# SqueezeAILab/SqueezeLLM

Measured on AMD Instinct MI355X. Metric: LLaMA-7B-shaped quantised-linear decode throughput (batch 1, all QuantLinearLUT matvecs of the model per token), higher is better.
Workload: dtype f32; 1 GPU; llama-7b w4 s0 (dense-only), batch=1 decode, 32 layers x 7 linears, op vecquant4matmul_nuq_perchannel; config_name=7b-w4-s0, launch=graph, linears sharing an input (q/k/v, gate/up) fused into one launch each, parallelism=single GPU, world_size=1, rccl_ranks=0

## Files before the change

### squeezellm_amd/csrc/sqllm_capi.hip

```cpp
#include <hip/hip_runtime.h>
#include <stdint.h>
#include <string.h>

#include <atomic>

#include "sqllm_hip.h"
#include "sqllm_host.h"
#include "sqllm_kernels.h"

namespace sqllm {
hipError_t (*g_launch_linear_gated)(int bits, const LaunchArgs& a, void* pair, hipStream_t stream) = nullptr;
hipError_t (*g_launch_linear_ep)(int bits, const LaunchArgs& a, const void* residual, int act, hipStream_t stream) = nullptr;
}

namespace sqllm_host {

ExperimentalHooks g_experimental;
static Knobs g_knobs[kMaxDevices];

int device_slot() {
  int dev = 0;
  if (hipGetDevice(&dev) != hipSuccess) {
    (void)hipGetLastError();
    dev = 0;
// ... 160 lines not shown
  const int resident = table > 3 ? table : 3;
  if (batch > 5 || total <= resident * cu_count() || (gm[0].sparse_last & 1)) return false;
  int sparse = 0;
  for (int i = 0; i < n; ++i) sparse += gm[i].csr_blocks + gm[i].topx_blocks;
  if (4 * sparse < 5 * cu_count()) return false;
  for (int i = 0; i < n; ++i)
    if (gm[i].csr_blocks > 0) {
      gm[i].csr_wide = 1;
      gm[i].csr_blocks = (gm[i].nnz + 2 * sqllm::kCsrChunk - 1) / (2 * sqllm::kCsrChunk);
      place_dense(&gm[i]);
    }
  return true;
}

void fill_segment(const sqllm_op* op, sqllm::Segment* sg) {
  sg->q = reinterpret_cast<const uint32_t*>(op->qweight);
  sg->y = op->mul;
  sg->lut = op->lookup_table;
  sg->rows = op->rows;
  sg->cols = op->cols;
  sg->vals = op->vals;
  sg->full_rows = op->topX > 0 ? op->full_rows : nullptr;
  sg->full_idx = op->topX > 0 ? op->full_row_indices : nullptr;
  sg->bias = nullptr;
  sg->out16 = nullptr;
}

static void cut_ranges(sqllm::KernelGeom* gm, int bits, int ops_in_launch, int step, int target, int grid_y) {
  const long long total_units = (long long)gm->col_tiles * gm->units_total;
  long long upw = (long long)opt(&Knobs::groups_per_wave) * step;
  bool aligned = false;
  if (upw <= 0) {
    if (opt(&Knobs::target_wgs) > 0) target = opt(&Knobs::target_wgs);
    target = (target + ops_in_launch - 1) / ops_in_launch;
    long long ranges = (target + grid_y - 1) / grid_y;
    if (ranges < 1) ranges = 1;
    upw = (total_units + ranges - 1) / ranges;
    const long long upws = (upw + step - 1) / step * step;
    const long long need = (gm->units_total + upws - 1) / upws;
    for (long long per_tile = need; per_tile >= 1 && per_tile >= need - 1 && !aligned; --per_tile) {
      long long even = (gm->units_total + per_tile - 1) / per_tile;
      even = (even + step - 1) / step * step;
      const long long n_even = (long long)gm->col_tiles * ((gm->units_total + even - 1) / even);
      if (n_even <= ranges && 10 * n_even >= 9 * ranges) { upw = even; aligned = true; }
    }
    if (aligned && ops_in_launch >= 3 && bits == 4 && gm->nnz > 0 && (gm->units_total + upw - 1) / upw == 3 &&
        gm->units_total % upw != 0 && gm->units_total % (2 * sqllm::kWaves) == 0)
      upw = gm->units_total / 2;
  }
  upw = (upw + step - 1) / step * step;
  if (upw > 0x3fffffff) upw = 0x3fffffff / step * step;
  gm->units_per_wg = (int)upw;
  gm->k_slices = (int)((gm->units_total + upw - 1) / upw);
  gm->dense_blocks = aligned ? gm->col_tiles * gm->k_slices : (int)((total_units + upw - 1) / upw);
  gm->sparse_last = 0;
  place_dense(gm);
}

void make_plan_mfma(const sqllm_op* op, sqllm::KernelGeom* gm, int ops_in_launch = 1, int row_blocks = 0, int wgs_per_cu = 0, int reserve = 0) {
  make_plan(op, gm, 1);
  const int mb = row_blocks > 0 ? row_blocks : sqllm::mfma_row_blocks(gm->batch);
  int target = (wgs_per_cu > 0 ? wgs_per_cu : mb == 4 ? 1 : 2) * cu_count();
  if (reserve > 0 && target - reserve >= target / 2) target -= reserve;
  cut_ranges(gm, op->bits, ops_in_launch, sqllm::kWaves * 4, target, (gm->batch + 16 * mb - 1) / (16 * mb));
}

constexpr int kWideTiles = 8;
int make_plan_wide(const sqllm_op* op, sqllm::KernelGeom* gm) {
  make_plan(op, gm, 1);
  const int row_blocks = (gm->batch + 63) / 64;
  const int col_groups = (gm->col_tiles + kWideTiles - 1) / kWideTiles;
  const long long units = (long long)col_groups * row_blocks;
  const int cus = cu_count();
  const long long full = units / cus * cus;
  const long long rem = units - full;
  int max_s = gm->units_total / (op->bits == 4 ? 32 : 8);
  if (max_s > sqllm::kMaxSlices) max_s = sqllm::kMaxSlices;
  if (max_s < 1) max_s = 1;
  int s = rem > 0 ? (int)(cus / rem) : 1;
  if (s > max_s) s = max_s;
  if (s < 1) s = 1;
  const int want = opt(&Knobs::groups_per_wave) * 4;
  int upw = want > 0 ? want : ((gm->units_total + s - 1) / s + 3) / 4 * 4;
  if (upw > gm->units_total) upw = (gm->units_total + 3) / 4 * 4;
  gm->units_per_wg = upw;
  gm->k_slices = (gm->units_total + upw - 1) / upw;
  const long long blocks = full + rem * gm->k_slices;
  gm->dense_blocks = blocks > 0x7fffffff ? 0x7fffffff : (int)blocks;
  gm->sparse_last = 0;
  place_dense(gm);
  return (int)full;
}

bool takes_wide_path(const sqllm_op* op, bool with_scratch, bool capturing) {
  if (!opt(&Knobs::mfma_split)) return false;
  const int from = opt(&Knobs::mfma_wide_min_batch);
  if (from > 0) return op->batch >= from;
  if (op->batch < 64) return false;
  if (with_scratch) {
    const double work = (double)op->batch * op->K * op->N;
    return work >= (op->bits == 4 ? 5.7e9 : 4e9) * (capturing ? 3.0 : 1.0);
  }
  const long long col_groups = ((op->N + sqllm::kTileN - 1) / sqllm::kTileN + kWideTiles - 1) / kWideTiles;
  const long long units = col_groups * ((op->batch + 63) / 64);
  return 5 * units >= 4 * (long long)cu_count();
}

void fold_csr_into_dense(sqllm::KernelGeom* gm) {
  gm->fold_csr = gm->nnz > 0 ? 1 : 0;
  gm->csr_blocks = 0;
  place_dense(gm);
}

int small_topx_blocks(const sqllm_op* op, bool with_xT, int ops_in_launch) {
  if (!(op->full_rows && op->topX > 0)) return 0;
  const int slabs = (op->K + sqllm::kTopxRows - 1) / sqllm::kTopxRows;
  if (!with_xT || op->topX > 16) return slabs;
  const int want = ops_in_launch == 1 ? (slabs <= 24 ? 24 : 16) : slabs <= 40 ? 8 : 16;
  return slabs < want ? slabs : want;
}

int small_wgs_per_cu_of(const sqllm_op* op) {
  const int v = opt(&Knobs::small_wgs_per_cu);
  return v > 0 ? v : 2;
}

int mfma_min_batch_of(const sqllm_op* op, int n_ops = 1) {
  const int v = opt(&Knobs::mfma_min_batch);
  if (v > 0) return v;
  if (op->bits != 4) return 9;
  const double mb = (double)op->K * op->N / 2e6;
  if (n_ops == 1 && mb <= 16.0) return 9;
  return 7;
}
int cols_max_batch_of(const sqllm_op* op) {
  const int v = opt(&Knobs::cols_max_batch);
  return v > 0 ? v : (op->bits == 3 ? 16 : ((double)op->K * op->N / 2e6 >= 20.0 ? 6 : 4));
}

bool takes_mfma_path(const sqllm_op* op, int n_ops = 1) { return op->batch >= 1 && op->batch >= mfma_min_batch_of(op, n_ops); }

bool takes_small_split(const sqllm_op* op, int n_ops = 1) {
  if (op->K >= (1 << 26)) return false;
  return takes_mfma_path(op, n_ops) && op->batch <= sqllm::kSmallSplitRows && opt(&Knobs::mfma_split) &&
         opt(&Knobs::mfma_fuse_small);
}

void make_plan_cols(const sqllm_op* op, sqllm::KernelGeom* gm, int ops_in_launch = 1) {
  make_plan(op, gm, 1);
  const int bt = sqllm::batch_tile_op(gm->batch);
  cut_ranges(gm, op->bits, ops_in_launch, sqllm::kWaves, 3 * cu_count(), (gm->batch + bt - 1) / bt);
}

int cols_min_batch_of() {
  const int v = opt(&Knobs::cols_min_batch);
  return v > 0 ? v : 2;
}

bool cols_pays(const sqllm_op* op, int n_ops) {
  if (opt(&Knobs::cols_min_batch) > 0 || opt(&Knobs::cols_max_batch) > 0) return true;
  const double mb = (double)op->K * op->N * op->bits / 8e6;
  if (op->bits == 4) return (n_ops >= 3 && op->batch <= 4 && !(op->batch == 2 && op->nnz > 0 && mb >= 32.0)) || (n_ops == 1 && mb >= 20.0);
  if (op->batch <= 4 && mb >= 16.0) return true;
  return op->N >= 8192;
}

bool cols_pays_batch1(const sqllm_op* sum, int n_ops, bool sparse) {
  const double mb = (double)sum->K * sum->N * sum->bits / 8e6;
  if (mb < 16.0) return false;
  if (!sparse) return n_ops >= 3 || (n_ops == 1 && sum->K >= 2ll * sum->N) || (n_ops == 2 && sum->bits == 3);
  return sum->K % 2048 == 0 && mb <= 40.0 && n_ops >= (sum->bits == 3 ? 2 : 3);
}

static bool op_has_sparse(const sqllm_op* op) { return (op->rows && op->nnz > 0) || (op->full_rows && op->topX > 0); }

static bool cols_route(const sqllm_op* sum, int n_ops, bool sparse) {
  const int b = sum->batch <= 0 ? 1 : sum->batch;
  const bool explicit_range = opt(&Knobs::cols_min_batch) > 0 || opt(&Knobs::cols_max_batch) > 0;
  if (b == 1 && !explicit_range) return cols_pays_batch1(sum, n_ops, sparse);
  return b >= cols_min_batch_of() && b <= cols_max_batch_of(sum) && cols_pays(sum, n_ops);
}

bool group_takes_cols_path(const sqllm_op* ops, int n) {
  sqllm_op sum = ops[0];
  long long N = 0;
  bool sparse = false;
  for (int i = 0; i < n; ++i) {
    N += ops[i].N;
    sparse = sparse || op_has_sparse(&ops[i]);
  }
  sum.N = N > 0x7fffffff ? 0x7fffffff : (int)N;
  return !takes_mfma_path(&ops[0], n) && cols_route(&sum, n, sparse);
}

bool takes_cols_path(const sqllm_op* op) { return !takes_mfma_path(op) && cols_route(op, 1, op_has_sparse(op)); }


enum Route {
  kFusedTiles,
  kFusedLinear,
  kColsGroup,
  kFusedSmall,
  kPerOpMfma,
  kPerOpCols,
};

static Route route_of(const sqllm_op* ops, int n, bool is_linear) {
  if (is_linear) return kFusedLinear;
  if (n > 1 && opt(&Knobs::cols_groups) && group_takes_cols_path(ops, n)) return kColsGroup;
  if (takes_small_split(&ops[0], n)) return kFusedSmall;
  if (takes_mfma_path(&ops[0], n)) return kPerOpMfma;
  if (n == 1 && takes_cols_path(&ops[0])) return kPerOpCols;
  return kFusedTiles;
}

static int validate_group(const sqllm_op* ops, int n, sqllm_stream_t stream, Route route) {
  const bool tiles = route == kFusedTiles || route == kFusedLinear;
  for (int i = 0; i < n; ++i) {
    const sqllm_op* op = &ops[i];
    int rc = validate(op);
    if (rc == SQLLM_OK) rc = validate_csr_values(op, stream);
    if (rc != SQLLM_OK) return rc;
    const bool same_batch = tiles ? (op->batch <= 0 ? 1 : op->batch) == (ops[0].batch <= 0 ? 1 : ops[0].batch) : op->batch == ops[0].batch;
    if (op->vec != ops[0].vec || op->K != ops[0].K || op->bits != ops[0].bits || !same_batch) return SQLLM_E_GROUP;
    if (!tiles && (uint64_t)op->batch * (uint64_t)op->K >= (1ull << 31)) return SQLLM_E_SHAPE;
  }
  return SQLLM_OK;
}

struct ScratchFacts {
  bool xT = false;
  bool planes = false;
  bool capturing = false;
};

struct LaunchPlan {
  int first = 0, n_seg = 0;
  int block0[sqllm::kMaxSegments + 1] = {};
  bool wide = false;
  int wide_full_units = 0;
  int row_blocks = 0;
  bool split = true;
  bool sparse_in_grid = false;
  bool sparse_launch = false;
};

struct GroupPlan {
  Route route = kFusedTiles;
  int rc = SQLLM_OK;
  int n_launches = 0;
  LaunchPlan launch[sqllm::kMaxSegments];
  sqllm::KernelGeom gm[sqllm::kMaxSegments];
};

static int layout_blocks(const sqllm::KernelGeom* gm, int n, bool pad, int* block0) {
  int at = 0;
  for (int i = 0; i < n; ++i) {
    block0[i] = at;
    at += pad ? padded_blocks(gm[i]) : gm[i].dense_block0 + gm[i].dense_blocks;
  }
  for (int i = n; i <= sqllm::kMaxSegments; ++i) block0[i] = at;
  return at;
}

static void plan_mfma_op(const sqllm_op* op, const ScratchFacts& f, LaunchPlan* lp, sqllm::KernelGeom* gm) {
  lp->split = opt(&Knobs::mfma_split) != 0;
  lp->wide = takes_wide_path(op, f.planes, f.capturing);
  if (lp->wide) lp->wide_full_units = make_plan_wide(op, gm);
  else make_plan_mfma(op, gm);
  const int sparse = gm->csr_blocks + gm->topx_blocks;
  const bool may_fuse = sparse > 0 && !lp->wide && lp->split && opt(&Knobs::mfma_fuse_sparse);
  lp->sparse_in_grid = may_fuse && (op->batch <= 32 || sparse < cu_count());
  if (may_fuse && !lp->sparse_in_grid && op->batch <= 64) {
    lp->row_blocks = 2;
    make_plan_mfma(op, gm, 1, 2);
    lp->sparse_in_grid = true;
  }
  lp->sparse_launch = sparse > 0 && !lp->sparse_in_grid;
}

static void plan_group(const sqllm_op* ops, int n, Route route, const ScratchFacts& f, GroupPlan* p) {
  p->route = route;
  const bool per_op = route == kPerOpMfma || route == kPerOpCols;
  switch (route) {
    case kColsGroup:
    case kPerOpCols:
      for (int i = 0; i < n; ++i) make_plan_cols(&ops[i], &p->gm[i], n);
      break;
    case kFusedSmall: {
      int reserve = 0;
      if (f.xT || opt(&Knobs::small_reserve_topx))
        for (int i = 0; i < n; ++i) reserve += round8(small_topx_blocks(&ops[i], f.xT, n));
      for (int i = 0; i < n; ++i) {
        make_plan_mfma(&ops[i], &p->gm[i], n, 0, small_wgs_per_cu_of(&ops[i]), reserve);
        p->gm[i].topx_blocks = small_topx_blocks(&ops[i], f.xT, n);
        fold_csr_into_dense(&p->gm[i]);
      }
      break;
    }
    case kPerOpMfma:
      for (int i = 0; i < n; ++i) plan_mfma_op(&ops[i], f, &p->launch[i], &p->gm[i]);
      break;
    case kFusedLinear:
      for (int i = 0; i < n; ++i) {
        const sqllm_op* op = &ops[i];
        sqllm::KernelGeom* gm = &p->gm[i];
        const int csr_bound = (op->rows && op->nnz > 0) ? op->K / sqllm::kCsrChunk + 2 : 0;
        make_plan(op, gm, n, sqllm::kMaxContrib - csr_bound > 1 ? sqllm::kMaxContrib - csr_bound : 1);
        gm->topx_blocks = 0;
        place_dense(gm);
        if (gm->k_slices + (gm->csr_blocks ? op->K / sqllm::kCsrChunk + 2 : 0) > sqllm::kMaxContrib) {
          p->rc = SQLLM_E_SHAPE;
          return;
        }
      }
      break;
    case kFusedTiles:
      for (int i = 0; i < n; ++i) make_plan(&ops[i], &p->gm[i], n);
      break;
  }
  p->n_launches = per_op ? n : 1;
  for (int l = 0; l < p->n_launches; ++l) {
    LaunchPlan* lp = &p->launch[l];
    lp->first = per_op ? l : 0;
    lp->n_seg = per_op ? 1 : n;
    const int total = layout_blocks(&p->gm[lp->first], lp->n_seg, !per_op, lp->block0);
    if (route != kFusedTiles) continue;
    const bool widened = widen_csr_chunks(p->gm, n, ops[0].bits, ops[0].batch, total);
    set_role_priority(p->gm, n, ops[0].bits, ops[0].batch, widened ? layout_blocks(p->gm, n, true, lp->block0) : total, widened);
  }
}

}

using namespace sqllm_host;

extern "C" {

int sqllm_abi_version(void) { return SQLLM_ABI_VERSION; }

const char* sqllm_error_string(int code) {
  switch (code) {
    case SQLLM_OK: return "ok";
    case SQLLM_E_BITS: return "bits must be 3 or 4";
    case SQLLM_E_SHAPE: return "bad shape: need K % 32 == 0, N % 4 == 0, height == K/32*bits, positive dims";
    case SQLLM_E_NULL: return "a required pointer is NULL";
    case SQLLM_E_ALIGN: return "qweight / lookup_table must be 16-byte aligned";
    case SQLLM_E_SPARSE: return "inconsistent sparse operands";
    case SQLLM_E_BATCH: return "bad batch / vec_height";
    case SQLLM_E_OPTION: return "unknown option or bad value";
    case SQLLM_E_GROUP: return "ops of a group must share vec, K, bits and batch (1..4 ops per group)";
    default: break;
  }
  if (code > 0) return hipGetErrorString(static_cast<hipError_t>(code));
  return "unknown sqllm error";
}

struct Option { const char* name; std::atomic<int> Knobs::*field; int max; };
static const Option kOptions[] = {
    {"target_wgs", &Knobs::target_wgs, 1 << 24},
    {"groups_per_wave", &Knobs::groups_per_wave, 1 << 24},
    {"cu_count", &Knobs::cu_count, 1 << 16},
    {"sparse_last", &Knobs::sparse_last, 1},
    {"cols_groups", &Knobs::cols_groups, 1},
    {"mfma_min_batch", &Knobs::mfma_min_batch, 0x7fffffff},
    {"cols_min_batch", &Knobs::cols_min_batch, 0x7fffffff},
    {"cols_max_batch", &Knobs::cols_max_batch, 0x7fffffff},
    {"sparse_transpose", &Knobs::sparse_transpose, 1},
    {"scratch_in_capture", &Knobs::scratch_in_capture, 1},
    {"validate_csr", &Knobs::validate_csr, 1},
    {"mfma_split", &Knobs::mfma_split, 1},
    {"split_planes_min_batch", &Knobs::split_planes_min_batch, 0x7fffffff},
    {"mfma_wide_min_batch", &Knobs::mfma_wide_min_batch, 0x7fffffff},
    {"mfma_fuse_small", &Knobs::mfma_fuse_small, 1},
    {"mfma_fuse_sparse", &Knobs::mfma_fuse_sparse, 1},
    {"scratch_pool_threshold", &Knobs::scratch_pool_threshold, 1},
    {"small_wgs_per_cu", &Knobs::small_wgs_per_cu, 8},
    {"small_reserve_topx", &Knobs::small_reserve_topx, 1},
    {"small_planes", &Knobs::small_planes, 1},
};
static const Option* find_option(const char* name) {
  for (const Option& o : kOptions)
    if (!strcmp(name, o.name)) return &o;
  return nullptr;
}

int sqllm_set_option(const char* name, int value) {
  if (!name || value < 0) return SQLLM_E_OPTION;
  if (const Option* o = find_option(name)) {
    if (value > o->max) return SQLLM_E_OPTION;
    (knobs().*(o->field)).store(value);
    return SQLLM_OK;
  }
  if (g_experimental.set_option) return g_experimental.set_option(name, value);
  return SQLLM_E_OPTION;
}

int sqllm_get_option(const char* name, int* value) {
  if (!name || !value) return SQLLM_E_OPTION;
  if (const Option* o = find_option(name)) {
    *value = (knobs().*(o->field)).load();
    return SQLLM_OK;
  }
  if (g_experimental.get_option) return g_experimental.get_option(name, value);
  return SQLLM_E_OPTION;
}

int sqllm_plan_query(const sqllm_op* op, sqllm_plan* plan) {
  if (!plan) return SQLLM_E_NULL;
  if (!op) return SQLLM_E_NULL;
  if (op->bits != 3 && op->bits != 4) return SQLLM_E_BITS;
  if (op->K <= 0 || op->N <= 0 || (op->K % 32) != 0 || (op->N % 4) != 0) return SQLLM_E_SHAPE;
  ScratchFacts facts;
  facts.xT = opt(&Knobs::sparse_transpose) != 0;
  facts.planes = true;
  GroupPlan p;
  plan_group(op, 1, route_of(op, 1, false), facts, &p);
  const sqllm::KernelGeom& gm = p.gm[0];
  const LaunchPlan& lp = p.launch[0];
  plan->col_tiles = gm.col_tiles;
  plan->k_slices = gm.k_slices;
  plan->groups_per_wave = gm.units_per_wg;
  plan->dense_blocks = gm.dense_blocks;
  plan->csr_blocks = gm.csr_blocks;
  plan->topx_blocks = gm.topx_blocks;
  const bool mfma = p.route == kPerOpMfma;
  plan->grid_x = mfma ? gm.dense_blocks : gm.dense_block0 + gm.dense_blocks;
  const int rows_per_pass = lp.wide ? gm.batch
                            : (mfma || p.route == kFusedSmall) ? 16 * (lp.row_blocks ? lp.row_blocks : sqllm::mfma_row_blocks(gm.batch))
                                                               : sqllm::batch_tile_op(gm.batch);
  plan->grid_y = (gm.batch + rows_per_pass - 1) / rows_per_pass;
  return SQLLM_OK;
}

static int64_t align16(int64_t v) { return (v + 15) / 16 * 16; }

int64_t sqllm_linear_workspace_bytes(const sqllm_op* op) {
  if (!op || op->N <= 0) return 0;
  return align16(8ll * (op->batch <= 0 ? 1 : op->batch) * op->N);
}

constexpr int kSplitPlanesMinBatch = 64;
struct WideScratch {
  void* block = nullptr;
  float* xT = nullptr;
  int Bp = 0;
  void* planes = nullptr;
  uint32_t* flags = nullptr;
  float* slabs = nullptr;
  bool capturing = false;
  hipStream_t s = nullptr;
  struct Layout { uint64_t xt = 0, planes = 0, flags = 0, slabs = 0; int Bp = 0; uint64_t total() const { return xt + planes + flags + slabs; } };
  static Layout layout(const sqllm_op* ops, int n, bool capturing) {
    Layout L;
    if (!ops || n < 1 || ops[0].batch <= 0 || ops[0].K <= 0) return L;
    bool any_csr = false, any_wide = false;
    uint64_t slab_bytes = 0;
    for (int i = 0; i < n; ++i) {
      any_csr = any_csr || (ops[i].nnz > 0 && ops[i].rows && ops[i].cols && ops[i].vals);
      if (validate(&ops[i]) != SQLLM_OK || !takes_wide_path(&ops[i], true, capturing)) continue;
      any_wide = true;
      sqllm::KernelGeom gm;
      const int full = make_plan_wide(&ops[i], &gm);
      const uint64_t b = sqllm::wide_slab_bytes(gm.dense_blocks, full, gm.k_slices);
      if (b > slab_bytes) slab_bytes = b;
    }
    const bool want_xT = any_csr && opt(&Knobs::sparse_transpose);
    int from = opt(&Knobs::split_planes_min_batch);
    if (from == 0) from = kSplitPlanesMinBatch;
    const uint64_t chunks = sqllm::split_planes_chunks(ops[0].batch, ops[0].K);
    const bool want_planes = any_wide && ops[0].batch >= from && chunks < (1ull << 31);
    if (!want_xT && !want_planes) return L;
    L.Bp = (ops[0].batch + 63) / 64 * 64;
    L.xt = want_xT ? (uint64_t)ops[0].K * L.Bp * sizeof(float) : 0;
    L.planes = want_planes ? chunks * 16 : 0;
    L.flags = want_planes ? (sqllm::kSplitFlagWgs * sizeof(uint32_t) + 15) / 16 * 16 : 0;
    L.slabs = want_planes ? slab_bytes : 0;
    return L;
  }
  int acquire(const sqllm_op* ops, int n, sqllm_stream_t stream, hipEvent_t* e0, void* ws, int64_t ws_bytes) {
    s = static_cast<hipStream_t>(stream);
    if (!ops[0].vec || ops[0].batch <= 0 || ops[0].K <= 0) return SQLLM_OK;
    bool in_capture = false;
    hipStreamCaptureStatus cs = hipStreamCaptureStatusNone;
    if (!(hipStreamIsCapturing(s, &cs) == hipSuccess && cs == hipStreamCaptureStatusNone)) {
      (void)hipGetLastError();
      in_capture = true;
    }
    char* p = nullptr;
    Layout L = layout(ops, n, false);
    if (ws && (reinterpret_cast<uintptr_t>(ws) & 15u) == 0 && L.total() > 0 && (uint64_t)(ws_bytes > 0 ? ws_bytes : 0) >= L.total()) {
      p = static_cast<char*>(ws);
    } else {
      capturing = in_capture;
      if (capturing && !opt(&Knobs::scratch_in_capture)) return SQLLM_OK;
      L = layout(ops, n, capturing);
      if (L.total() == 0) return SQLLM_OK;
      keep_scratch_in_pool();
      if (hipMallocAsync(&block, L.total(), s) != hipSuccess || !block) {
        (void)hipGetLastError();
        block = nullptr;
        return SQLLM_OK;
      }
      p = static_cast<char*>(block);
    }
    if (L.total() == 0) return SQLLM_OK;
    if (L.xt) {
      xT = reinterpret_cast<float*>(p);
      Bp = L.Bp;
      const hipError_t e = sqllm::transpose_vec(ops[0].vec, xT, ops[0].batch, ops[0].K, Bp, s, e0 ? *e0 : nullptr);
      if (e != hipSuccess) return static_cast<int>(e);
      if (e0) *e0 = nullptr;
    }
    if (L.planes) {
      planes = p + L.xt;
      flags = reinterpret_cast<uint32_t*>(p + L.xt + L.planes);
      if (L.slabs) slabs = reinterpret_cast<float*>(p + L.xt + L.planes + L.flags);
// ... 456 lines not shown
```

### squeezellm_amd/csrc/sqllm_host.h

```cpp
#pragma once
#include <hip/hip_runtime.h>

#include <atomic>

#include "sqllm_hip.h"
#include "sqllm_kernels.h"

namespace sqllm_host {

struct Knobs {
  std::atomic<int> target_wgs{0};
  std::atomic<int> groups_per_wave{0};
  std::atomic<int> cu_count{0};
  std::atomic<int> sparse_last{0};
  std::atomic<int> cols_groups{1};
  std::atomic<int> mfma_min_batch{0};
  std::atomic<int> cols_min_batch{0};
  std::atomic<int> cols_max_batch{0};
  std::atomic<int> scratch_in_capture{1};
  std::atomic<int> sparse_transpose{1};
  std::atomic<int> validate_csr{0};
  std::atomic<int> mfma_split{1};
  std::atomic<int> scratch_pool_threshold{1};
  std::atomic<int> mfma_wide_min_batch{0};
  std::atomic<int> split_planes_min_batch{0};
  std::atomic<int> mfma_fuse_sparse{1};
  std::atomic<int> mfma_fuse_small{1};
  std::atomic<int> small_reserve_topx{0};
  std::atomic<int> small_planes{1};
  std::atomic<int> small_wgs_per_cu{0};
};
constexpr int kMaxDevices = 32;

int device_slot();
Knobs& knobs();
int cu_count();
int validate(const sqllm_op* op);
int validate_sparse(const sqllm_op* op);
int validate_csr_values(const sqllm_op* op, sqllm_stream_t stream);
void make_plan(const sqllm_op* op, sqllm::KernelGeom* gm, int ops_in_launch = 1, int max_slices = sqllm::kMaxSlices,
               int waves = sqllm::kWaves);
void fill_segment(const sqllm_op* op, sqllm::Segment* sg);

struct ExperimentalHooks {
  int (*set_option)(const char* name, int value) = nullptr;
  int (*get_option)(const char* name, int* value) = nullptr;
  bool (*route)(const sqllm_op* ops, int n, sqllm_stream_t stream, hipEvent_t e0, hipEvent_t e1, int* rc) = nullptr;
  void (*decorate)(sqllm::LaunchArgs* a) = nullptr;
  int (*csr_ablation_bits)() = nullptr;
  bool (*skip_prepare_small)() = nullptr;
};
extern ExperimentalHooks g_experimental;

}
```

### squeezellm_amd/csrc/sqllm_kernels.h

```cpp
#pragma once
#include <hip/hip_runtime.h>
#include <stdint.h>

#ifndef SQLLM_ABLATION_BUILD
#if defined(SQLLM_PAIR3) || defined(SQLLM_PAIR3_NOCONFLICT) || defined(SQLLM_MFMA_VAR) || defined(SQLLM_MFMA_FAKE) || \
    defined(SQLLM_HALF_STAGES) || defined(SQLLM_WAVES) || defined(SQLLM_STREAM_RING) || defined(SQLLM_STREAM_WGCU) || \
    defined(SQLLM_STREAM_PRO) || defined(SQLLM_TOPX_ROWS) || defined(SQLLM_CSR_CHUNK)
#error "kernel variant switches need -DSQLLM_ABLATION_BUILD (python -m squeezellm_amd.build --ablation)"
#endif
#endif
#ifndef SQLLM_WAVES
#define SQLLM_WAVES 8
#endif
#ifndef SQLLM_CSR_CHUNK
#define SQLLM_CSR_CHUNK 1024
#endif
#ifndef SQLLM_TOPX_ROWS
#define SQLLM_TOPX_ROWS 256
#endif

namespace sqllm {

constexpr int kWaves = SQLLM_WAVES;
constexpr int kTileN = 64;
constexpr int kCsrChunk = SQLLM_CSR_CHUNK;
constexpr int kCsrSpanMax = 2048;
constexpr int kCsrEdge = 256;
constexpr int kCsrXtSpan = 191;
constexpr int kSparsePassRows = 128;
constexpr int kTopxRows = SQLLM_TOPX_ROWS;
constexpr int kTopxLds = 1024;
constexpr int kMaxBatchTile = 8;
constexpr int kMaxSlices = 120;
constexpr int kMaxContrib = 63;

constexpr int cmax(int a, int b) { return a > b ? a : b; }
constexpr int lds_floats(int lut_entries, int waves, int bt, bool pair3 = false) {
  return cmax((pair3 ? 4 * 64 * 32 : 4 * lut_entries * 32) + waves * bt * kTileN + 4 + bt * kTileN,
              cmax(2 * kCsrSpanMax, kTopxLds));
}

struct KernelGeom {
  int K, N, batch;
  int col_tiles;
  int units_total;
  int units_per_wg;
  int k_slices;
  int dense_blocks;
  int dense_block0;
  int csr_blocks;
  int topx_blocks;
  int nnz, topX;
  int sparse_last;
  int fold_csr;
  int csr_wide;
  int dense_prio;
};

constexpr int kMaxSegments = 4;

struct Segment {
  const uint32_t* q;
  float* y;
  const float* lut;
  const int* rows;
  const int* cols;
  const float* vals;
  const float* full_rows;
  const int* full_idx;
  const float* bias;
  void* out16;
  KernelGeom gm;
};

struct GroupArgs {
  int n_seg;
  int block0[kMaxSegments + 1];
  Segment seg[kMaxSegments];
};

struct LaunchArgs {
  const void* x;
  bool linear = false;
  bool bf16 = false;
  GroupArgs ga;
  hipEvent_t ev_start = nullptr;
  hipEvent_t ev_stop = nullptr;
  int ablate = 0;
  int lds_pad = 0;
  const float* xT = nullptr;
  int Bp = 0;
  const void* planes = nullptr;
  const uint32_t* plane_flags = nullptr;
  bool wide = false;
  int wide_full_units = 0;
  float* wide_slabs = nullptr;
  int row_blocks = 0;
};

inline int batch_tile(int batch) { return batch <= 1 ? 1 : batch == 2 ? 2 : batch <= 4 ? 4 : 8; }
inline int batch_tile_op(int batch) { return (batch == 3 || batch == 5 || batch == 6 || batch == 7) ? batch : batch_tile(batch); }

inline int mfma_row_blocks(int batch) { return batch <= 16 ? 1 : batch <= 32 ? 2 : 4; }

hipError_t launch_fused(int bits, const LaunchArgs& a, hipStream_t stream);
hipError_t launch_linear_bf16(int bits, const LaunchArgs& a, hipStream_t stream);
extern bool (*g_fused_variant)(int bits, const LaunchArgs& a, hipStream_t stream, hipError_t* err);
extern hipError_t (*g_launch_linear_gated)(int bits, const LaunchArgs& a, void* pair, hipStream_t stream);
extern hipError_t (*g_launch_linear_ep)(int bits, const LaunchArgs& a, const void* residual, int act, hipStream_t stream);
hipError_t launch_batched_mfma(int bits, const LaunchArgs& a, hipStream_t stream);
hipError_t launch_batched_mfma_split(int bits, const LaunchArgs& a, hipStream_t stream);
hipError_t launch_batched_mfma_split_all(int bits, const LaunchArgs& a, hipStream_t stream);
hipError_t launch_batched_mfma_wide(int bits, const LaunchArgs& a, hipStream_t stream);
hipError_t launch_batched_cols(int bits, const LaunchArgs& a, hipStream_t stream);
constexpr int kSplitFlagWgs = 256;
inline uint64_t split_planes_chunks(int batch, int K) { return (uint64_t)((batch + 63) / 64 * 4) * (uint64_t)(K / 32 + 1) * 192u; }
inline uint64_t wide_slab_bytes(int dense_blocks, int full_units, int k_slices) {
  return k_slices > 1 ? (uint64_t)(dense_blocks - full_units) * 8u * 64u * 64u * 4u : 0;
}
hipError_t split_vec(const float* x, void* planes, uint32_t* flags, int batch, int K, hipStream_t stream, hipEvent_t ev_start);
constexpr int kSmallSplitRows = 16;
hipError_t launch_small_split(int bits, const LaunchArgs& a, hipStream_t stream);
hipError_t transpose_vec(const float* x, float* xT, int batch, int K, int Bp, hipStream_t stream, hipEvent_t ev_start);
constexpr int small_rows_log2(int batch) { return batch <= 2 ? 1 : batch <= 4 ? 2 : batch <= 8 ? 3 : 4; }
hipError_t transpose_small(const float* x, float* xT, int batch, int K, hipStream_t stream, hipEvent_t ev_start);
hipError_t prepare_small(const float* x, float* xT, void* planes, int batch, int K, hipStream_t stream, hipEvent_t ev_start);
inline int64_t small_planes_bytes(int K) { return (int64_t)(K / 32 + 1) * 3072; }
inline int64_t transpose_small_bytes(int batch, int K) { return ((int64_t)K << small_rows_log2(batch)) * 4; }
hipError_t launch_batched_sparse(const LaunchArgs& a, hipStream_t stream);
hipError_t check_csr(const int* rows, int N, int nnz, hipStream_t stream, int* bad);

}
```

### squeezellm_amd/csrc/sqllm_kernels.hip

```cpp
#include "sqllm_fused.h"
#include "sqllm_split_common.h"

namespace sqllm {

bool (*g_fused_variant)(int bits, const LaunchArgs& a, hipStream_t stream, hipError_t* err) = nullptr;

constexpr int kXtStride = 36;
constexpr int mfma_codebook_floats(int bits) { return bits == 4 ? 2 * 4096 / 4 : 4 * 8 * 128 / 4; }
constexpr int mfma_lds_floats(int bits, int mb, int waves) {
  return mfma_codebook_floats(bits) + cmax(waves * 16 * mb * kXtStride, waves * 16 * 64);
}

template <int BITS, int MB, int WAVES>
__device__ __forceinline__ void dense_role_mfma(const float* __restrict__ x, const u32x4* __restrict__ q,
                                                float* __restrict__ y, const float* __restrict__ lut, int K, int N,
                                                int batch, int m0, int bid, int n_col_tiles, int units_total,
                                                int units_per_wg, int units_stride, float* lds) {
  using F = Fmt<BITS>;
  constexpr int L = F::kLut, R = F::kRows, KU = F::kK;
  constexpr int NPH = KU / 8;
  constexpr int TR = 16 * MB;
  constexpr int XL = TR / 8;
  constexpr int ESTRIDE = (BITS == 4) ? 256 : 128;
  constexpr int SUBB = (BITS == 4) ? (L * ESTRIDE) / 2 : L * ESTRIDE;
// ... 188 lines not shown
  using P1 = std::integral_constant<int, 1>;
  using P2 = std::integral_constant<int, 2>;
  using P3 = std::integral_constant<int, 3>;
  auto decode_group = [&](int g, const u32x4 (&w)[R], f32x4 (&xcur)[XL], u32x4 (&wn)[R], f32x4 (&xn)[XL]) {
    load_w(g + 1, wn);
    float v[4][8];
    if constexpr (NPH == 1) {
      load_x(g + 1, 0, xn);
      if (!(SQLLM_MFMA_VAR & 2)) __builtin_amdgcn_sched_barrier(0);
      lookups(w, P0{}, v);
      phase(v, xcur, g);
    } else {
      f32x4 xo[XL];
      load_x(g, 1, xo);
      if (!(SQLLM_MFMA_VAR & 2)) __builtin_amdgcn_sched_barrier(0);
      lookups(w, P0{}, v);
      phase(v, xcur, g);
      load_x(g, 2, xcur);
      if (!(SQLLM_MFMA_VAR & 2)) __builtin_amdgcn_sched_barrier(0);
      lookups(w, P1{}, v);
      phase(v, xo, g);
      load_x(g, 3, xo);
      if (!(SQLLM_MFMA_VAR & 2)) __builtin_amdgcn_sched_barrier(0);
      lookups(w, P2{}, v);
      phase(v, xcur, g);
      load_x(g + 1, 0, xn);
      if (!(SQLLM_MFMA_VAR & 2)) __builtin_amdgcn_sched_barrier(0);
      lookups(w, P3{}, v);
      phase(v, xo, g);
    }
    if (!(SQLLM_MFMA_VAR & 2)) __builtin_amdgcn_sched_barrier(0);
  };
  for (int g = 0; g < n_g; g += 2) {
    decode_group(g, wa, xa, wb, xb);
    decode_group(g + 1, wb, xb, wa, xa);
  }

  __syncthreads();
  float* slab = slabs + wave * (16 * 64) + (4 * grp) * 64 + 4 * i16;
#pragma unroll
  for (int mb = 0; mb < MB; ++mb) {
    if (mb) __syncthreads();
    *reinterpret_cast<f32x4*>(slab + 0 * 64) = f32x4{acc[mb][0].x, acc[mb][1].x, acc[mb][2].x, acc[mb][3].x};
    *reinterpret_cast<f32x4*>(slab + 1 * 64) = f32x4{acc[mb][0].y, acc[mb][1].y, acc[mb][2].y, acc[mb][3].y};
    *reinterpret_cast<f32x4*>(slab + 2 * 64) = f32x4{acc[mb][0].z, acc[mb][1].z, acc[mb][2].z, acc[mb][3].z};
    *reinterpret_cast<f32x4*>(slab + 3 * 64) = f32x4{acc[mb][0].w, acc[mb][1].w, acc[mb][2].w, acc[mb][3].w};
    __syncthreads();
#pragma unroll
    for (int e = tid; e < 16 * 64; e += WAVES * 64) {
      const int r = m0 + 16 * mb + (e >> 6);
      const int col = col0 + (e & 63);
      float sum = 0.f;
#pragma unroll
      for (int w = 0; w < WAVES; ++w) sum += slabs[w * (16 * 64) + e];
      if (r < batch && col < N) acc_add(y + (size_t)r * N + col, sum);
    }
  }
  }
}

template <int BITS, int MB, int WAVES>
__global__ void __launch_bounds__(WAVES * 64, (BITS == 4 && MB <= 2 && !(SQLLM_MFMA_VAR & 256)) ? 4 : 1)
sqllm_fused_batched(const float* x, const GroupArgs ga) {
  __shared__ __attribute__((aligned(16))) float lds[mfma_lds_floats(BITS, MB, WAVES)];
  const Segment sg = ga.seg[0];
  asm volatile("" ::SQLLM_SEG_OPERANDS(sg), "s"(x));
  __builtin_amdgcn_sched_barrier(0);
  const KernelGeom& gm = sg.gm;
  const int m0 = blockIdx.y * 16 * MB;
  dense_role_mfma<BITS, MB, WAVES>(x, reinterpret_cast<const u32x4*>(sg.q), sg.y, sg.lut, gm.K, gm.N, gm.batch, m0,
                                   (int)blockIdx.x, gm.col_tiles, gm.units_total, gm.units_per_wg, units_stride_of(gm), lds);
}

template <int WAVES>
__global__ void __launch_bounds__(WAVES * 64)
sqllm_sparse_batched(const float* x, const GroupArgs ga, const float* xT, int Bp, int pass_rows) {
  constexpr int T = WAVES * 64;
  __shared__ __attribute__((aligned(16))) float lds[kWideSparseLdsFloats];
  const Segment sg = ga.seg[0];
  asm volatile("" ::SQLLM_SEG_OPERANDS(sg), "s"(x));
  __builtin_amdgcn_sched_barrier(0);
  const KernelGeom& gm = sg.gm;
  const int sp = blockIdx.x;
  const int m0 = blockIdx.y * pass_rows;
  int rows_here = gm.batch - m0;
  if (rows_here > pass_rows) rows_here = pass_rows;
  if (sp < gm.csr_blocks) {
    if (xT) {
      csr_role<T, 1, float, float, true>(x, sg.y, sg.rows, sg.cols, sg.vals, gm.nnz, gm.K, gm.N, m0, rows_here, sp, lds, nullptr, 0, xT, Bp, SQLLM_PROBE_PTR(sg));
    } else {
      constexpr int CBT = 32;
      for (int bb = 0; bb < rows_here; bb += CBT) {
        if (bb) __syncthreads();
        csr_role<T, CBT, float, float>(x, sg.y, sg.rows, sg.cols, sg.vals, gm.nnz, gm.K, gm.N, m0 + bb,
                                       rows_here - bb < CBT ? rows_here - bb : CBT, sp, lds, nullptr, 0);
      }
    }
  } else if (sp < gm.csr_blocks + gm.topx_blocks) {
    for (int bb = 0; bb < rows_here; bb += 64) {
      if (bb) __syncthreads();
      topx_role<T, float, float, false, NoGate, 8>(x, sg.y, sg.full_rows, sg.full_idx, gm.topX, gm.K, gm.N, m0 + bb, rows_here - bb < 64 ? rows_here - bb : 64,
                                 sp - gm.csr_blocks, lds);
    }
  }
}

typedef float f32x8 __attribute__((ext_vector_type(8)));
constexpr int cols_table_floats(int bits) { return bits == 4 ? 17 * 64 : 65 * 64 * 2; }
constexpr int cols_lds_floats(int bits, int bt, int waves) {
  return cmax(cols_table_floats(bits) + waves * bt * 64, cmax(2 * kCsrSpanMax, kTopxLds));
}
constexpr int cols_stage_k(int bt) { return bt * 8 <= 32 ? 8 : 4; }

__device__ __forceinline__ uint32_t field6_x512(uint32_t t0, uint32_t t1, uint32_t t2, int M) {
  const int bit = 6 * M, w = bit >> 5, o = bit & 31;
  const uint32_t lo = (w == 0) ? t0 : (w == 1) ? t1 : t2;
  uint32_t f;
  if (o <= 26) {
    if (o > 9) f = lo >> (o - 9);
    else if (o < 9) f = lo << (9 - o);
    else f = lo;
  } else {
    const uint32_t hi = (w == 0) ? t1 : t2;
    f = __builtin_amdgcn_alignbit(hi, lo, o) << 9;
  }
  return f & 0x7E00u;
}

typedef const __attribute__((address_space(4))) float* cfloatp;
typedef const __attribute__((address_space(4))) char* ccharp;
template <int ST> struct XVec;
template <> struct XVec<4> {
  typedef f32x4 type;
  static __device__ __forceinline__ type load(ccharp base, uint32_t off) {
    return *reinterpret_cast<const __attribute__((address_space(4))) type*>(base + off);
  }
};
template <> struct XVec<8> {
  typedef f32x8 type;
  static __device__ __forceinline__ type load(ccharp base, uint32_t off) {
    return *reinterpret_cast<const __attribute__((address_space(4))) type*>(base + off);
  }
};

template <int BITS, int BT, int WAVES>
__device__ __forceinline__ void dense_role_cols(const float* __restrict__ x, const uint32_t* __restrict__ q,
                                                float* __restrict__ y, const float* __restrict__ lut, int K, int N,
                                                int b0, int nb, int bid, int n_col_tiles, int units_total,
                                                int units_per_wg, int units_stride, float* lds) {
  using F = Fmt<BITS>;
  constexpr int L = F::kLut, R = F::kRows, KU = F::kK;
  constexpr int ST = cols_stage_k(BT);
  constexpr int SPU = KU / ST;
  constexpr int D = BITS == 4 ? 4 : 2;
  constexpr int NB = 2;
  constexpr int NS = D * SPU;
  constexpr int NP = ST / 2;
  constexpr int NA = BT >= 4 ? 1 : 4 / BT;
  using XV = typename XVec<ST>::type;
  static_assert(NS % 2 == 0, "stages alternate between two register sets");
  static_assert(WAVES == 8, "table build assumes 8 waves");
  __builtin_amdgcn_s_waitcnt(0);
  const int tid = threadIdx.x, lane = tid & 63;
  const int w = __builtin_amdgcn_readfirstlane(tid >> 6);
  char* table = reinterpret_cast<char*>(lds);
  float* slabs = lds + cols_table_floats(BITS);
  const uint32_t lane_base = BITS == 4 ? (4u * lane) | 0x1000u : 8u * lane;
  const uint32_t row_bytes = 4u * (uint32_t)N;
  ccharp xrow[BT];
#pragma unroll
  for (int b = 0; b < BT; ++b) xrow[b] = reinterpret_cast<ccharp>(reinterpret_cast<uintptr_t>(x + (size_t)(b0 + (b < nb ? b : nb - 1)) * K));
  uint32_t soff[D][R];
#pragma unroll
  for (int j = 0; j < D; ++j)
#pragma unroll
    for (int r = 0; r < R; ++r) soff[j][r] = (uint32_t)(j * WAVES * R + r) * row_bytes;
  if constexpr (BITS == 4) { if (tid < 64) *reinterpret_cast<float*>(table + 16 * 256 + 4 * tid) = 0.f; }
  else { if (tid < 64) *reinterpret_cast<f32x2*>(table + 64 * 512 + 8 * tid) = f32x2{0.f, 0.f}; }

  const unsigned total = (unsigned)n_col_tiles * (unsigned)units_stride;
  unsigned gpos = (unsigned)bid * (unsigned)units_per_wg;
  unsigned gend = gpos + (unsigned)units_per_wg;
  if (gend > total) gend = total;
  bool first = true;
  while (gpos < gend) {
    const int ct = __builtin_amdgcn_readfirstlane((int)(gpos / (unsigned)units_stride));
    const int u0 = (int)(gpos - (unsigned)ct * (unsigned)units_stride);
    if (u0 >= units_total) { gpos = (unsigned)(ct + 1) * (unsigned)units_stride; continue; }
    int u1 = units_total;
    if ((unsigned)(u1 - u0) > gend - gpos) u1 = u0 + (int)(gend - gpos);
    gpos += (unsigned)(u1 - u0);
    if (u1 == units_total) gpos = (unsigned)(ct + 1) * (unsigned)units_stride;
    const int col0 = ct * kTileN;
    const int col = col0 + lane;
    const int colc = col < N ? col : N - 1;
    const float* lp = lut + (size_t)colc * L;
    float tv[8];
    float thi = 0.f;
    if constexpr (BITS == 4) {
      const f32x2 t = *reinterpret_cast<const f32x2*>(lp + 2 * w);
      tv[0] = t.x; tv[1] = t.y;
    } else {
      const f32x4 ta = *reinterpret_cast<const f32x4*>(lp), tb2 = *reinterpret_cast<const f32x4*>(lp + 4);
      tv[0] = ta.x; tv[1] = ta.y; tv[2] = ta.z; tv[3] = ta.w; tv[4] = tb2.x; tv[5] = tb2.y; tv[6] = tb2.z; tv[7] = tb2.w;
      thi = lp[w];
    }
    const int n_units = u1 - u0;
    const int n_w = n_units > w ? (n_units - w + WAVES - 1) / WAVES : 0;
    const int nc = (n_w + D - 1) / D;
    const __amdgpu_buffer_rsrc_t qrsrc =
        __builtin_amdgcn_make_buffer_rsrc(const_cast<uint32_t*>(q), 0, (uint32_t)(u1 * R) * row_bytes, 0x00020000);
    uint32_t voff[NB];
#pragma unroll
    for (int k = 0; k < NB; ++k) voff[k] = 4u * (uint32_t)colc + (uint32_t)((u0 + w + k * D * WAVES) * R) * row_bytes;
    auto load_chunk = [&](int k, uint32_t (&dst)[D][R]) {
#pragma unroll
      for (int j = 0; j < D; ++j)
#pragma unroll
        for (int r = 0; r < R; ++r) dst[j][r] = __builtin_amdgcn_raw_buffer_load_b32(qrsrc, voff[k], soff[j][r], 2 );
      voff[k] += (uint32_t)(NB * D * WAVES * R) * row_bytes;
    };
    uint32_t wbuf[NB][D][R];
#pragma unroll
    for (int k = 0; k < NB; ++k) load_chunk(k, wbuf[k]);
    asm volatile("" ::: "memory");
    __builtin_amdgcn_sched_barrier(0);
    if (!first) __syncthreads();
    first = false;
    if constexpr (BITS == 4) {
      *reinterpret_cast<float*>(table + (2 * w) * 256 + 4 * lane) = tv[0];
      *reinterpret_cast<float*>(table + (2 * w + 1) * 256 + 4 * lane) = tv[1];
    } else {
#pragma unroll
      for (int i0 = 0; i0 < 8; ++i0) *reinterpret_cast<f32x2*>(table + (8 * w + i0) * 512 + lane_base) = f32x2{tv[i0], thi};
    }
    __syncthreads();

    f32x2 acc[BT][NA];
#pragma unroll
    for (int b = 0; b < BT; ++b)
#pragma unroll
      for (int a = 0; a < NA; ++a) acc[b][a] = f32x2{0.f, 0.f};
    struct St { f32x2 v[NP]; XV x[BT]; };
    auto issue = [&](const uint32_t (&buf)[D][R], int st, int cc, St& o) {
      const int j = st / SPU, sub = st % SPU;
      const int i = cc * D + j;
      const bool live = i < n_w;
      if constexpr (BITS == 4) {
        const uint32_t lo = buf[j][0] & 0x0F0F0F0Fu, hi = (buf[j][0] >> 4) & 0x0F0F0F0Fu;
#define SQ_L(WORD, SEL) *reinterpret_cast<const float __attribute__((address_space(3)))*>(__builtin_amdgcn_perm(WORD, lane_base, SEL))
#pragma unroll
        for (int m = 0; m < NP; ++m) {
          const uint32_t sel = live ? 0x0C0C0400u + ((uint32_t)(sub * NP + m) << 8) : 0x0C0C0100u;
          o.v[m] = f32x2{SQ_L(lo, sel), SQ_L(hi, sel)};
        }
#undef SQ_L
      } else {
        const uint32_t lane_or_dead = lane_base | (live ? 0u : 0x8000u);
#pragma unroll
        for (int m = 0; m < NP; ++m)
          o.v[m] = *reinterpret_cast<const f32x2 __attribute__((address_space(3)))*>(
              lane_or_dead | field6_x512(buf[j][0], buf[j][1], buf[j][2], sub * NP + m));
      }
      int u = u0 + w + i * WAVES;
      if (u > u1 - 1) u = u1 - 1;
      uint32_t koff = 4u * (uint32_t)(u * KU + sub * ST);
      asm volatile("" : "+s"(koff));
#pragma unroll
      for (int b = 0; b < BT; ++b) o.x[b] = XVec<ST>::load(xrow[b], koff);
    };
    auto fmas = [&](const St& o) {
#pragma unroll
      for (int m = 0; m < NP; ++m)
#pragma unroll
        for (int b = 0; b < BT; ++b)
          acc[b][m % NA] = __builtin_elementwise_fma(o.v[m], f32x2{o.x[b][2 * m], o.x[b][2 * m + 1]}, acc[b][m % NA]);
    };
    if constexpr (BT == 1) {
      constexpr int GS = 32 / ST;
      constexpr int LPS = BITS == 4 ? 2 * NP : NP;
      static_assert(NS % GS == 0 && (NB * NS / GS) % 2 == 0, "vec groups alternate between two SGPR sets");
      struct V { f32x2 v[NP]; };
      XV xs[2][GS];
      auto look = [&](const uint32_t (&buf)[D][R], int st, int cc, V& o, auto guard) {
        const int j = st / SPU, sub = st % SPU;
        bool live = true;
        if constexpr (decltype(guard)::value) live = cc * D + j < n_w;
        if constexpr (BITS == 4) {
          const uint32_t lo = buf[j][0] & 0x0F0F0F0Fu, hi = (buf[j][0] >> 4) & 0x0F0F0F0Fu;
#define SQ_L(WORD, SEL) *reinterpret_cast<const float __attribute__((address_space(3)))*>(__builtin_amdgcn_perm(WORD, lane_base, SEL))
#pragma unroll
          for (int m = 0; m < NP; ++m) {
            const uint32_t sel = live ? 0x0C0C0400u + ((uint32_t)(sub * NP + m) << 8) : 0x0C0C0100u;
            o.v[m] = f32x2{SQ_L(lo, sel), SQ_L(hi, sel)};
          }
#undef SQ_L
        } else {
          const uint32_t lane_or_dead = lane_base | (live ? 0u : 0x8000u);
#pragma unroll
          for (int m = 0; m < NP; ++m)
            o.v[m] = *reinterpret_cast<const f32x2 __attribute__((address_space(3)))*>(
                lane_or_dead | field6_x512(buf[j][0], buf[j][1], buf[j][2], sub * NP + m));
        }
      };
      auto vec_group = [&](int st0, int cc, XV (&xg)[GS]) {
#pragma unroll
        for (int g = 0; g < GS; ++g) {
          const int j = (st0 + g) / SPU, sub = (st0 + g) % SPU;
// ... 324 lines not shown
```

Measured before the change: 824.1 tokens/s.

## Model cols-kernel slot waste to pick batch-1 K-split cuts and routing

Adds a host-side cost model that counts padded per-wave work slots for the column kernel, given its chunk size and chunks-in-flight. At batch 1 it re-cuts the K ranges per workgroup to a wave-aligned length that minimises wasted slots, but only when the current plan crosses tile boundaries or a new knob asks for it. Two-op 4-bit groups such as gate/up are now routed to the cols path when the cut wastes under about 5% of slots. This targets idle lanes and uneven tail work in decode matvecs, at the cost of more planning logic and a possible change in workgroup counts.

New measurement: 905.6 tokens/s, median of 6. 1.1x the previous value.

```diff
diff --git a/squeezellm_amd/csrc/sqllm_capi.hip b/squeezellm_amd/csrc/sqllm_capi.hip
--- a/squeezellm_amd/csrc/sqllm_capi.hip
+++ b/squeezellm_amd/csrc/sqllm_capi.hip
@@ -336,6 +336,63 @@
   cut_ranges(gm, op->bits, ops_in_launch, sqllm::kWaves, 3 * cu_count(), (gm->batch + bt - 1) / bt);
 }
 
+static long long cols_piece_slots(int bits, long long n) {
+  const int D = sqllm::cols_chunk_units(bits), NB = sqllm::kColsChunksInFlight, W = sqllm::kWaves;
+  auto wave = [&](long long n_w) { return (long long)NB * D * (((n_w + D - 1) / D + NB - 1) / NB); };
+  return (n % W) * wave(n / W + 1) + (W - n % W) * wave(n / W);
+}
+static long long cols_tile_slots(int bits, int U, int L) {
+  const int k = (U + L - 1) / L;
+  return (k - 1) * cols_piece_slots(bits, L) + cols_piece_slots(bits, U - (long long)(k - 1) * L);
+}
+static long long cols_plan_slots(int bits, const sqllm::KernelGeom& gm, bool* crossing) {
+  const long long U = gm.units_total, L = gm.units_per_wg, total = gm.col_tiles * U;
+  if (gm.dense_blocks == gm.col_tiles * gm.k_slices) return gm.col_tiles * cols_tile_slots(bits, (int)U, (int)L);
+  *crossing = true;
+  return total / L * cols_piece_slots(bits, L) + cols_piece_slots(bits, total % L);
+}
+
+static int best_aligned_cut(int bits, int U, long long tiles, long long sparse, long long* slots_per_tile) {
+  const int W = sqllm::kWaves;
+  const long long room = 4ll * cu_count() - sparse, want = 3ll * cu_count();
+  int best = 0, prev = 0;
+  long long best_slots = 0;
+  for (int p = 1; p <= U; ++p) {
+    const int L = ((U + p - 1) / p + W - 1) / W * W;
+    if (L == prev) continue;
+    prev = L;
+    const long long k = (U + L - 1) / L, wgs = tiles * k;
+    if (wgs > room || tiles * k * L >= (1ll << 31)) break;
+    const long long slots = cols_tile_slots(bits, U, L);
+    if (!best || slots < best_slots || (slots == best_slots && wgs <= want)) { best = L; best_slots = slots; }
+    if (L == W) break;
+  }
+  *slots_per_tile = best_slots;
+  return best;
+}
+
+static void cut_ranges_one_row(const sqllm_op* ops, sqllm::KernelGeom* gm, int n) {
+  if (opt(&Knobs::groups_per_wave) > 0 || opt(&Knobs::target_wgs) > 0) return;
+  const int bits = ops[0].bits, U = gm[0].units_total;
+  long long tiles = 0, sparse = 0, today = 0;
+  bool crossing = false;
+  for (int i = 0; i < n; ++i) {
+    tiles += gm[i].col_tiles;
+    sparse += gm[i].dense_block0;
+    today += cols_plan_slots(bits, gm[i], &crossing);
+  }
+  const bool by_slots = opt(&Knobs::cols_slot_cut) != 0;
+  if (!crossing && !by_slots) return;
+  long long slots = 0;
+  const int L = best_aligned_cut(bits, U, tiles, sparse, &slots);
+  if (!L || tiles * slots > today) return;
+  for (int i = 0; i < n; ++i) {
+    gm[i].units_per_wg = L;
+    gm[i].k_slices = (U + L - 1) / L;
+    gm[i].dense_blocks = gm[i].col_tiles * gm[i].k_slices;
+  }
+}
+
 int cols_min_batch_of() {
   const int v = opt(&Knobs::cols_min_batch);
   return v > 0 ? v : 2;
@@ -349,19 +406,34 @@
   return op->N >= 8192;
 }
 
-bool cols_pays_batch1(const sqllm_op* sum, int n_ops, bool sparse) {
+bool cols_pays_batch1(const sqllm_op* sum, int n_ops, bool sparse, const sqllm_op* ops) {
   const double mb = (double)sum->K * sum->N * sum->bits / 8e6;
   if (mb < 16.0) return false;
-  if (!sparse) return n_ops >= 3 || (n_ops == 1 && sum->K >= 2ll * sum->N) || (n_ops == 2 && sum->bits == 3);
+  if (!sparse) {
+    if (n_ops >= 3 || (n_ops == 1 && sum->K >= 2ll * sum->N) || (n_ops == 2 && sum->bits == 3)) return true;
+    if (n_ops != 2 || opt(&Knobs::groups_per_wave) > 0 || opt(&Knobs::target_wgs) > 0) return false;
+    for (int i = 0; i < 2; ++i)
+      if (ops[i].bits != 4 || ops[i].K != ops[0].K || ops[i].K <= 0 || ops[i].N <= 0 || ops[i].K % 32 != 0 || ops[i].N % 4 != 0) return false;
+    sqllm::KernelGeom gm[2];
+    for (int i = 0; i < 2; ++i) make_plan_cols(&ops[i], &gm[i], 2);
+    cut_ranges_one_row(ops, gm, 2);
+    long long slots = 0, units = 0;
+    bool crossing = false;
+    for (int i = 0; i < 2; ++i) {
+      slots += cols_plan_slots(4, gm[i], &crossing);
+      units += (long long)gm[i].col_tiles * gm[i].units_total;
+    }
+    return !crossing && 100 * units >= 95 * slots;
+  }
   return sum->K % 2048 == 0 && mb <= 40.0 && n_ops >= (sum->bits == 3 ? 2 : 3);
 }
 
 static bool op_has_sparse(const sqllm_op* op) { return (op->rows && op->nnz > 0) || (op->full_rows && op->topX > 0); }
 
-static bool cols_route(const sqllm_op* sum, int n_ops, bool sparse) {
+static bool cols_route(const sqllm_op* sum, int n_ops, bool sparse, const sqllm_op* ops) {
   const int b = sum->batch <= 0 ? 1 : sum->batch;
   const bool explicit_range = opt(&Knobs::cols_min_batch) > 0 || opt(&Knobs::cols_max_batch) > 0;
-  if (b == 1 && !explicit_range) return cols_pays_batch1(sum, n_ops, sparse);
+  if (b == 1 && !explicit_range) return cols_pays_batch1(sum, n_ops, sparse, ops);
   return b >= cols_min_batch_of() && b <= cols_max_batch_of(sum) && cols_pays(sum, n_ops);
 }
 
@@ -374,10 +446,10 @@
     sparse = sparse || op_has_sparse(&ops[i]);
   }
   sum.N = N > 0x7fffffff ? 0x7fffffff : (int)N;
-  return !takes_mfma_path(&ops[0], n) && cols_route(&sum, n, sparse);
-}
-
-bool takes_cols_path(const sqllm_op* op) { return !takes_mfma_path(op) && cols_route(op, 1, op_has_sparse(op)); }
+  return !takes_mfma_path(&ops[0], n) && cols_route(&sum, n, sparse, ops);
+}
+
+bool takes_cols_path(const sqllm_op* op) { return !takes_mfma_path(op) && cols_route(op, 1, op_has_sparse(op), op); }
 
 
 enum Route {
@@ -470,6 +542,10 @@
     case kColsGroup:
     case kPerOpCols:
       for (int i = 0; i < n; ++i) make_plan_cols(&ops[i], &p->gm[i], n);
+      if (p->gm[0].batch == 1) {
+        if (route == kColsGroup) cut_ranges_one_row(ops, p->gm, n);
+        else for (int i = 0; i < n; ++i) cut_ranges_one_row(&ops[i], &p->gm[i], 1);
+      }
       break;
     case kFusedSmall: {
       int reserve = 0;
@@ -547,6 +623,7 @@
     {"cu_count", &Knobs::cu_count, 1 << 16},
     {"sparse_last", &Knobs::sparse_last, 1},
     {"cols_groups", &Knobs::cols_groups, 1},
+    {"cols_slot_cut", &Knobs::cols_slot_cut, 1},
     {"mfma_min_batch", &Knobs::mfma_min_batch, 0x7fffffff},
     {"cols_min_batch", &Knobs::cols_min_batch, 0x7fffffff},
     {"cols_max_batch", &Knobs::cols_max_batch, 0x7fffffff},
diff --git a/squeezellm_amd/csrc/sqllm_host.h b/squeezellm_amd/csrc/sqllm_host.h
--- a/squeezellm_amd/csrc/sqllm_host.h
+++ b/squeezellm_amd/csrc/sqllm_host.h
@@ -14,6 +14,7 @@
   std::atomic<int> cu_count{0};
   std::atomic<int> sparse_last{0};
   std::atomic<int> cols_groups{1};
+  std::atomic<int> cols_slot_cut{0};
   std::atomic<int> mfma_min_batch{0};
   std::atomic<int> cols_min_batch{0};
   std::atomic<int> cols_max_batch{0};
diff --git a/squeezellm_amd/csrc/sqllm_kernels.h b/squeezellm_amd/csrc/sqllm_kernels.h
--- a/squeezellm_amd/csrc/sqllm_kernels.h
+++ b/squeezellm_amd/csrc/sqllm_kernels.h
@@ -33,6 +33,11 @@
 constexpr int kMaxBatchTile = 8;
 constexpr int kMaxSlices = 120;
 constexpr int kMaxContrib = 63;
+
+constexpr int kColsChunksInFlight = 2;
+constexpr int cols_chunk_units(int bits) { return bits == 4 ? 4 : 2; }
+constexpr int cols_wave_quantum(int bits) { return kColsChunksInFlight * cols_chunk_units(bits); }
+constexpr int cols_quantum(int bits) { return cols_wave_quantum(bits) * kWaves; }
 
 constexpr int cmax(int a, int b) { return a > b ? a : b; }
 constexpr int lds_floats(int lut_entries, int waves, int bt, bool pair3 = false) {
diff --git a/squeezellm_amd/csrc/sqllm_kernels.hip b/squeezellm_amd/csrc/sqllm_kernels.hip
--- a/squeezellm_amd/csrc/sqllm_kernels.hip
+++ b/squeezellm_amd/csrc/sqllm_kernels.hip
@@ -364,8 +364,8 @@
   constexpr int L = F::kLut, R = F::kRows, KU = F::kK;
   constexpr int ST = cols_stage_k(BT);
   constexpr int SPU = KU / ST;
-  constexpr int D = BITS == 4 ? 4 : 2;
-  constexpr int NB = 2;
+  constexpr int D = cols_chunk_units(BITS);
+  constexpr int NB = kColsChunksInFlight;
   constexpr int NS = D * SPU;
   constexpr int NP = ST / 2;
   constexpr int NA = BT >= 4 ? 1 : 4 / BT;
```
